# David-OConnor/molchanica

Hardware: AMD Instinct MI355X
Metric: MD atom-updates/sec (and steps/sec), 1M-atom solvated box (higher is better)
Workload: dtype f32

## Files before the change

### molchanica_amd/csrc/mdx_api.hip

```cpp
#include "mdx_comm.h"
#include <algorithm>
#include <atomic>
#include <chrono>
#include <cfloat>
#include <cmath>
#include <cstring>
#include <dlfcn.h>
#include <mutex>
#include <unordered_map>

static thread_local std::string g_last_error;
void mdx_set_error(const std::string& s) { g_last_error = s; }

static inline unsigned div_up(unsigned a, unsigned b) { return (a + b - 1) / b; }
static bool cut_on(float rc) { return rc > 0.f && std::isfinite(rc); }
static uint32_t f2u(float f) { uint32_t u; std::memcpy(&u, &f, 4); return u; }
static float u2f(uint32_t u) { float f; std::memcpy(&f, &u, 4); return f; }

#define FAIL(code, msg) do { mdx_set_error(msg); return (code); } while (0)

template <typename T>
static int upload_vec(T** dptr, const std::vector<T>& v, hipStream_t st) {
    if (*dptr) { (void)hipFree(*dptr); *dptr = nullptr; }
    HIP_TRY(hipMalloc((void**)dptr, std::max<size_t>(sizeof(T) * v.size(), 16)));
// ... 1277 lines not shown
    HIP_TRY(hipStreamSynchronize(h->stream));
    mdx_prof_collect(h);
    h->profile = enable != 0; h->profile_level = enable;
    if (enable) {
        h->stats.nb_ms_sum = h->stats.bonded_ms_sum = h->stats.integ_ms_sum = 0.0;
        h->stats.rebuild_ms_sum = h->stats.wall_ms_sum = 0.0;
        h->stats.nb_launches = h->stats.bonded_launches = h->stats.integ_launches = 0;
        if (h->dd) for (int k = 0; k < MDX_DIAG_PHASES; ++k) { h->dd->phase_ms[k] = 0.0; h->dd->phase_n[k] = 0; }
    }
    return MDX_OK;
}

extern "C" int mdx_get_skin(const mdx_handle* h, float* skin, int* tuning) {
    if (!h) FAIL(MDX_EPARAM, "null handle");
    if (skin) *skin = h->cfg.skin;
    if (tuning) *tuning = (h->skin_tune.on && h->skin_tune.phase < 4) ? 1 : 0;
    return MDX_OK;
}

extern "C" int mdx_pair_launch_info(const mdx_handle* h, uint32_t out[24]) {
    if (!h || !out) FAIL(MDX_EPARAM, "null argument");
    for (int k = 0; k < 8; ++k) { out[k] = h->pair_info_step[k]; out[8 + k] = h->pair_info_any[k]; }
    out[16] = h->inner_rebuilds; out[17] = h->inner_from_rebuild ? 1u : 0u; out[18] = h->water_step_launches; out[19] = h->water_step_mixed_launches;
    out[20] = (uint32_t)h->onepass_launches; out[21] = (uint32_t)h->onepass_violations; out[22] = 0u; out[23] = 0u;
    return MDX_OK;
}

extern "C" int mdx_get_stats(mdx_handle* h, mdx_stats* out) {
    if (!h || !out) FAIL(MDX_EPARAM, "null argument");
    HIP_TRY(hipSetDevice(h->device));
    HIP_TRY(hipStreamSynchronize(h->stream));
    mdx_prof_collect(h);
    h->stats.step_count = h->step_count; h->stats.rebuild_count = h->rebuild_count;
    h->stats.n_inner_cluster_pairs = 0; h->stats.prune_passes = 0;
    if (h->d.inner_count) {
        unsigned long long c[MDX_EPART + 1];
        HIP_TRY(hipSetDevice(h->device));
        HIP_TRY(hipMemcpyAsync(c, h->d.inner_count, sizeof(c), hipMemcpyDeviceToHost, h->stream));
        HIP_TRY(hipStreamSynchronize(h->stream));
        unsigned long long tot = 0;
        for (int k = 0; k < MDX_EPART; ++k) tot += c[k];
        h->stats.prune_passes = c[MDX_EPART];
        h->stats.n_inner_cluster_pairs = c[MDX_EPART] ? tot / c[MDX_EPART] : 0;
    }
    h->stats.n_owned = h->dd ? h->dd->n_owned : h->n_local;
    h->stats.n_ghost = h->dd ? h->dd->n_local - h->dd->n_owned : 0;
    h->stats.repartitions = h->dd ? h->dd->repartitions : 0;
// ... 300 lines not shown
```

### molchanica_amd/csrc/mdx_grid.hip

```cpp
#include "mdx_internal.h"
#include <atomic>
#include <chrono>
#include <algorithm>
#include <cfloat>
#include <cmath>

#define WAVE_LDS_SYNC()                                      \
    do {                                                     \
        __builtin_amdgcn_fence(__ATOMIC_SEQ_CST, "workgroup"); \
        __builtin_amdgcn_wave_barrier();                     \
    } while (0)

static inline unsigned div_up(unsigned a, unsigned b) { return (a + b - 1) / b; }

constexpr int SCAN_THREADS = 256;
constexpr int SCAN_ITEMS = 8;
constexpr int SCAN_TILE = SCAN_THREADS * SCAN_ITEMS;

__device__ __forceinline__ uint32_t block_exclusive_scan_256(uint32_t v, uint32_t* s_wave, uint32_t* total) {
    const int lane = threadIdx.x & 63, wave = threadIdx.x >> 6;
    uint32_t inc = v;
#pragma unroll
    for (int d = 1; d < 64; d <<= 1) {
        uint32_t t = __shfl_up(inc, d);
// ... 985 lines not shown
            if ((lane & 7) == 0 && newy != ent.y) entries[e0 + c * 8 + (lane >> 3)].y = newy;
            if (inner_on && (lane & 7) == 0) pin.entries_in[e0 + c * 8 + (lane >> 3)] = make_uint2(ent.x, newy_in);
        } else {
            const bool alive = (lane & 7) == 0 && ((newy >> 8) & 0xFFu) != 0u;
            const unsigned long long bal = __ballot(alive);
            if (alive) {
                const uint32_t rank = __popcll(bal & ((1ull << lane) - 1ull));
                entries[e0 + cnt.n_masked + wcur + rank] = make_uint2(ent.x, newy);
            }
            wcur += __popcll(bal);
            if (inner_on) {
                const bool alive_in = (lane & 7) == 0 && ((newy_in >> 8) & 0xFFu) != 0u;
                const unsigned long long bin = __ballot(alive_in);
                if (alive_in) pin.entries_in[e0 + cnt.n_masked + wcur_in + __popcll(bin & ((1ull << lane) - 1ull))] = make_uint2(ent.x, newy_in);
                wcur_in += __popcll(bin);
            }
        }
    }
    const uint32_t np_pad = (wcur + 7u) & ~7u;
    if (lane < (int)(np_pad - wcur)) entries[e0 + cnt.n_masked + wcur + lane] = make_uint2(null_cluster, 13u);
    if (inner_on) {
        const uint32_t nin_pad = (wcur_in + 7u) & ~7u;
        if (lane < (int)(nin_pad - wcur_in)) pin.entries_in[e0 + cnt.n_masked + wcur_in + lane] = make_uint2(null_cluster, 13u);
        if (lane == 0) pin.inner_nch[(size_t)t * 8] = nmc + (nin_pad >> 3);
    }
    const bool any_ghost = __any(ghost_hit);
    if (lane == 0) {
        counts[t].n_plain = np_pad;
        if (kept) atomicAdd(pc_slot(pair_count, t, 1), (unsigned long long)kept);
        if (tile_int) tile_int[t] = (!any_ghost && t * MDX_CL_PER_TILE < first_ghost_cluster) ? 1u : 0u;
    }
}

template <int W>
__global__ __launch_bounds__(W * 64) void prune_list_mw_kernel(uint32_t T, float r2, float shx, float shy, float shz,
                                                               const float4* __restrict__ posq, ListCounts* __restrict__ counts,
                                                               const uint32_t* __restrict__ entry_off, uint2* __restrict__ entries,
                                                               uint32_t null_cluster, unsigned long long* __restrict__ pair_count,
                                                               const uint32_t* __restrict__ rb_ctl, uint32_t* __restrict__ tile_int,
                                                               const uint8_t* __restrict__ cl_kind) {
    __shared__ float4 s_j[W][64];
    __shared__ uint32_t s_ghost;
    const int lane = threadIdx.x & 63, wave = __builtin_amdgcn_readfirstlane(threadIdx.x >> 6);
    uint32_t first_ghost_cluster = 0xFFFFFFFFu;
    if (rb_ctl) {
        T = __builtin_amdgcn_readfirstlane(rb_ctl[0]); null_cluster = T * MDX_CL_PER_TILE;
        first_ghost_cluster = __builtin_amdgcn_readfirstlane(rb_ctl[1]) * MDX_CL_PER_TILE;
// ... 953 lines not shown
    }
    const uint32_t T = h->T, S = h->S, NC = (T + 1) * MDX_CL_PER_TILE;
    {
        const TileOrderPlan plan = tile_order_plan(h, T);
        if (!res.classified) {
            h->tile_split = false; h->n_interior = 0;
            if (plan.split) MDX_TRY(mdx_classify_tiles(h, plan.lpt));
        }
        if (!res.ordered) {
            h->tile_lpt_on = false;
            if (plan.lpt) MDX_TRY(mdx_order_tiles_by_length(h, plan.grouped));
        }
    }
    h->list_valid = true;
    h->forces_valid = false;
    h->rebuild_count++; h->steps_since_rebuild = 0;
    mdx_dd_note_rebuild(h);
    h->inner_skin = h->inner_skin_auto > 0.f ? h->inner_skin_auto : c_inner_skin(h->cfg);
    h->dual_on = !h->dual_auto_off && mdx_nb_half(h) && prune && h->inner_skin > 0.f && h->inner_skin < h->cfg.skin &&
                 (h->n_vsites == 0 || h->vsites_convex);
    h->prune_pending = !(res.inner_built && h->dual_on);
    h->inner_from_rebuild = !h->prune_pending;
    if (h->inner_from_rebuild) ++h->inner_rebuilds;
    if (!d.inner_count) { ALLOC(d.inner_count, MDX_EPART + 8); HIP_TRY(hipMemsetAsync(d.inner_count, 0, sizeof(unsigned long long) * (MDX_EPART + 8), st)); }
    uint64_t nmask = (uint64_t)MC * 8;
    h->stats.n_atoms = N; h->stats.n_slots = S; h->stats.n_tiles = T; h->stats.n_clusters = NC;
    h->stats.n_list_entries = E; h->stats.n_masked_entries = nmask;
    h->stats.n_cluster_pairs = (mdx_nb_variant(h) >= 2) ? npairs : (uint64_t)E * 8;
    if (h->profile) {
        float ms = 0.f;
        HIP_TRY(hipEventRecord(e1, st)); HIP_TRY(hipEventSynchronize(e1));
        HIP_TRY(hipEventElapsedTime(&ms, e0, e1));
        h->stats.rebuild_ms_sum += ms;
        h->ev_pool.push_back(e0); h->ev_pool.push_back(e1);
    }
    return MDX_OK;
}

__global__ __launch_bounds__(1024) void lpt_order_kernel(uint32_t T, const ListCounts* __restrict__ counts, const uint32_t* __restrict__ is_int,
                                                         uint32_t* __restrict__ order, uint32_t group_tiles) {
    constexpr uint32_t NB = 8 * LPT_BUCKETS;
    __shared__ uint32_t s_hist[NB], s_cur[NB];
    for (uint32_t b = threadIdx.x; b < NB; b += blockDim.x) s_hist[b] = 0;
    __syncthreads();
    auto bucket = [&](uint32_t t) {
        const uint32_t nch = (counts[t].n_masked + counts[t].n_plain) >> 3;
// ... 143 lines not shown
```

### molchanica_amd/csrc/mdx_internal.h

```cpp
#pragma once
#include <hip/hip_runtime.h>
#include <stdint.h>
#include <chrono>
#include <string>
#include <vector>
#include "../../include/mdx.h"

#define MDX_TILE 64
#define MDX_CLUSTER 8
#define MDX_CL_PER_TILE 8
#define MDX_ACC_CONV 418.4f
#define MDX_KB 0.0019872041
#define MDX_INVALID 0xFFFFFFFFu
#define MDX_DUMMY_BASE 1.0e6f
#define MDX_DUMMY_STEP 64.0f
#define MDX_MAX_CHUNK 64
#define MDX_MAX_GROUPS 255

#define MDX_ESTRIDE 5
#define MDX_EPART 256
enum { EN_BOND = 0, EN_ANGLE, EN_DIHEDRAL, EN_LJ, EN_COUL, EN_LJ14, EN_COUL14, EN_KIN, EN_RECIP, EN_VIRIAL, EN_POSRE, EN_POSRE_VIR, EN_COUNT };

struct GridParams {
    float lo[3];
    float len[3];
    float inv_col[2];
// ... 270 lines not shown
        float dt_tuned = 0.f;
        std::chrono::steady_clock::time_point t0;
    } skin_tune;
    int chunk_s = -1;
    bool list_valid = false;
    bool forces_valid = false;
    bool in_slot_space = false;
    bool have_ext = false;
    uint64_t step_count = 0, rebuild_count = 0;
    bool profile = false; int profile_level = 0; bool prof_open = false;
    struct EvPair { hipEvent_t a, b; int kind; int tag; hipStream_t st; };
    int prof_tag = -1;
    uint32_t prof_seq = 0; bool prof_sampled = false;
    std::vector<EvPair> ev_pending;
    std::vector<hipEvent_t> ev_pool;
    mdx_stats stats{};
    int tstat_kind = 0; float tstat_temp = 300.f, tstat_tau = 1.f; uint32_t tstat_every = 10;
    int integrator = 0; float lang_gamma = 1.f, lang_temp = 300.f; uint64_t lang_seed = 0, lang_step = 0;
    int baro_kind = 0; float baro_p0 = 1.f, baro_tau = 5.f, baro_beta = 4.5e-5f; uint32_t baro_every = 25;
    double last_pressure = 0.0, last_mu = 1.0;
    bool force_zeroed = false;
    bool cons_full_kick = false;
    bool bonded_fused = false;
    uint32_t pair_info_step[8] = {}, pair_info_any[8] = {};
    bool bonded_deferred = false;
    uint64_t rng_state = 0;
    bool zero_com = false;
    uint32_t snap_every = 0; bool snap_vel = false;
    uint32_t snap_handlers[MDX_SNAP_HANDLERS] = {};
    double time_ps = 0.0;
    struct Snapshot { double time; uint64_t step; mdx_energies e; std::vector<float> pos, vel, frc; std::vector<mdx_hbond> hbonds; std::vector<float> between; uint32_t handler_mask = 0;
                      std::vector<double> foreign; };
    uint32_t water_first = 0, n_waters = 0, water_sites = 0;
    std::vector<uint8_t> hb_heavy; float hb_dmax = 2.5f, hb_angle_min = 120.f;
    std::vector<uint32_t> hb_donor_of;
    std::vector<uint32_t> h_bond_pairs;
    std::vector<Snapshot> snapshots;
    DeviceState d;
    StepCtl* h_ctl = nullptr;
    uint32_t ctl_seq = 0;
    uint32_t* h_rb = nullptr;
    uint32_t rb_seq = 0;
    uint32_t scan_gen = 0;
    bool cell_count_clean = false;
    bool slot_of_clean = false;
};
// ... 60 lines not shown
static inline bool mdx_nb_half(const mdx_handle* h) { return mdx_nb_variant(h) == 5; }
static inline uint32_t mdx_wpt8_below(const mdx_handle* h) {
    static const int env = [] { const char* e = std::getenv("MDX_WPT8_BELOW"); return e ? std::atoi(e) : -1; }();
    (void)h;
    return env >= 0 ? (uint32_t)env : 2048u;
}

#ifndef MDX_NB_WAVES
#define MDX_NB_WAVES 1
#endif
struct WptRule { int env; uint32_t wpt8_below; int decomposed; };
__host__ __device__ static inline int mdx_wpt_rule(const WptRule& r, uint32_t T) {
    if (r.env) return r.env;
    if (T >= 12000u) return r.decomposed ? 2 : 1;
    if (T >= (r.decomposed ? 8000u : 3000u)) return 2;
    return T < r.wpt8_below ? 8 : 4;
}
static inline WptRule mdx_wpt_rule_of(const mdx_handle* h) {
    static const int env = [] { const char* e = std::getenv("MDX_WPT"); return (e && (e[0] == '1' || e[0] == '2' || e[0] == '4' || e[0] == '8')) ? e[0] - '0' : 0; }();
    WptRule r; r.env = env; r.wpt8_below = mdx_wpt8_below(h); r.decomposed = (h->dd || h->n_local != h->N) ? 1 : 0;
    return r;
}
static inline int mdx_nb_wpt_half(const mdx_handle* h, uint32_t T) { return mdx_wpt_rule(mdx_wpt_rule_of(h), T); }

int mdx_build_constraints(mdx_handle* h, const mdx_system* s);
int mdx_remap_constraints(mdx_handle* h);
int mdx_launch_constrain_positions(mdx_handle* h, float dt, const uint32_t* d_gate, uint32_t* d_disp_out, uint32_t thr,
                                   uint32_t* d_prune_out = nullptr, bool skip_wstep = false);
int mdx_launch_constrain_velocities(mdx_handle* h, const uint32_t* d_gate, uint32_t thr);
bool mdx_water_step_ok(const mdx_handle* h);
bool mdx_water_step_mixed(const mdx_handle* h);
int mdx_launch_water_step(mdx_handle* h, int mode, float dt, const uint32_t* d_gate, uint32_t* d_disp_out, uint32_t thr, uint32_t* d_prune_out);
int mdx_launch_vsite_construct(mdx_handle* h, const uint32_t* d_gate, uint32_t thr);
int mdx_launch_constraint_virial(mdx_handle* h);
int mdx_check_box(const mdx_handle* h, const float* lo, const float* hi);
int mdx_launch_vsite_spread(mdx_handle* h, const uint32_t* d_gate, uint32_t thr);

int mdx_pme_setup(mdx_handle* h);
int mdx_pme_cu_split(const mdx_handle* h, const mdx_config* c);
int mdx_stream_create_masked(hipStream_t* s, int cus_per_xcd, bool complement);
int mdx_stream_unmask(mdx_handle* h);
void mdx_pme_destroy(mdx_handle* h);
int mdx_launch_pme(mdx_handle* h, bool energy, const uint32_t* d_gate, uint32_t thr);
int mdx_pme_fork(mdx_handle* h);
int mdx_pme_join(mdx_handle* h, const uint32_t* d_gate, uint32_t thr);

// ... 37 lines not shown
```

### molchanica_amd/csrc/mdx_nonbonded.hip

```cpp
#include "mdx_internal.h"
#include "mdx_bonded_dev.h"
#include "mdx_pair_dev.h"
#include <algorithm>
#include <cfloat>
#include <cstdlib>
#include <cstring>
#include <vector>

template <bool ENERGY, int COUL>
void launch_variant(mdx_handle* h, const NbArgs& a, bool geom, bool samecut);
#define NB_EXTERN(E, C) extern template void launch_variant<E, C>(mdx_handle*, const NbArgs&, bool, bool);
NB_EXTERN(false, CM_SHIFTED) NB_EXTERN(false, CM_RF) NB_EXTERN(false, CM_EWALD) NB_EXTERN(false, CM_SOFT)
NB_EXTERN(false, CM_EWALD_TAB)
NB_EXTERN(true, CM_SHIFTED) NB_EXTERN(true, CM_RF) NB_EXTERN(true, CM_EWALD) NB_EXTERN(true, CM_SOFT)
#undef NB_EXTERN

static bool cut_on(float rc) { return rc > 0.f && std::isfinite(rc); }
#define FAIL_NB(msg) do { mdx_set_error(msg); return MDX_EDEVICE; } while (0)

void mdx_fill_nb_params(const mdx_handle* h, NbParams& p, int* mode_out, bool* geom_out, bool* samecut_out) {
    const mdx_config& c = h->cfg;
    p.rc2_lj = cut_on(c.lj_cutoff) ? c.lj_cutoff * c.lj_cutoff : FLT_MAX;
    p.rc2_coul = cut_on(c.coulomb_cutoff) ? c.coulomb_cutoff * c.coulomb_cutoff : FLT_MAX;
    for (int d = 0; d < 3; ++d) p.shift[d] = h->per[d] ? (h->box_hi[d] - h->box_lo[d]) : 0.f;
    const bool ccut = cut_on(c.coulomb_cutoff);
    const float rc = c.coulomb_cutoff;
    p.alpha = c.ewald_alpha; p.soft2 = c.softening_sq;
    p.k_rf = 0.f; p.k_rf2 = 0.f; p.coul_shift = 0.f;
    p.alch_scale = h->alch_on ? (float)(1.0 - h->alch_lambda) : 1.0f;
    p.sc_alpha = h->alch_on ? h->sc_alpha : 0.f; p.sc_al = h->alch_on ? (float)(h->sc_alpha * h->alch_lambda) : 0.f;
    p.sc_sigmin = h->sc_sigma_min;
    int mode = CM_SHIFTED;
    switch (c.coulomb_mode) {
    case MDX_COULOMB_REACTION:
        mode = CM_RF;
        if (ccut) { p.k_rf = 1.0f / (2.0f * rc * rc * rc); p.k_rf2 = 2.0f * p.k_rf; p.coul_shift = 1.5f / rc; }
        break;
    case MDX_COULOMB_EWALD: mode = CM_EWALD; break;
// ... 140 lines not shown
```

### molchanica_amd/csrc/mdx_nonbonded_impl.h

```cpp
#pragma once
#include "mdx_internal.h"
#include "mdx_bonded_dev.h"
#include "mdx_pair_dev.h"
#include <algorithm>
#include <cfloat>
#include <cstdlib>
#include <type_traits>

constexpr int NB_WAVES = MDX_NB_WAVES;
#ifndef NB_ASM_PAIR
#define NB_ASM_PAIR 0
#endif
#ifndef NB_HALF_FLUSH
#define NB_HALF_FLUSH 0
#endif

template <bool BIAS, bool R2OUT>
__device__ __forceinline__ void pair_eval_asm(float xi, float yi, float zi, float qi, float sgi, float epi, const float4 pj,
                                              const float2 lj, float rc2, float bias, float& fx, float& fy, float& fz,
                                              float& g0, float& g1, float& g2, float& r2_out) {
    float dx, dy, dz, r2, t1, t2, t3, t4;
    if (BIAS) {
        asm volatile(
            "v_sub_f32 %[dy], %[yi], %[yj]\n\t"
            "v_sub_f32 %[dx], %[xi], %[xj]\n\t"
            "v_fma_f32 %[r2], %[dy], %[dy], %[bias]\n\t"
            "v_sub_f32 %[dz], %[zi], %[zj]\n\t"
            "v_fmac_f32 %[r2], %[dx], %[dx]\n\t"
            "v_fmac_f32 %[r2], %[dz], %[dz]\n\t"
            : [dx] "=&v"(dx), [dy] "=&v"(dy), [dz] "=&v"(dz), [r2] "=&v"(r2)
            : [xi] "v"(xi), [yi] "v"(yi), [zi] "v"(zi), [xj] "v"(pj.x), [yj] "v"(pj.y), [zj] "v"(pj.z), [bias] "v"(bias));
    } else {
// ... 124 lines not shown
        if (lane == 0) {
            double* q = a.energy + EN_COUNT + 8 + MDX_ESTRIDE * (blk & (MDX_EPART - 1));
            atomicAdd(q, 0.5 * elj); atomicAdd(q + 1, 0.5 * ecoul); atomicAdd(q + 2, 0.5 * evir);
        }
    }
}

template <int CTRL>
__device__ __forceinline__ float dpp_xadd(float v) {
    return v + __int_as_float(__builtin_amdgcn_update_dpp(0, __float_as_int(v), CTRL, 0xF, 0xF, true));
}

template <bool ENERGY, int COUL, bool GEOM, bool SAMECUT, int WPT, bool HALF, bool ALCH, int DUAL, int BW, bool STEP = false>
__device__ __forceinline__ void nb_cluster_body(const NbArgs& a, const bool owned_prune, float4 (*s_xyzq)[64], float2 (*s_lj)[64],
                                                float (*s_red)[3][64], float (*s_ownj)[64], float4 (*s_g)[64],
                                                unsigned long long (*s_mask)[64], const float4* __restrict__ etab = nullptr) {
    const int lane = threadIdx.x & 63, wave = __builtin_amdgcn_readfirstlane(threadIdx.x >> 6);
    constexpr int SPLIT = BW < WPT ? WPT / BW : 1;
    static_assert(SPLIT == 1 || HALF, "a tile split over workgroups returns its i-forces through atomics");
    constexpr int TPB = SPLIT > 1 ? 1 : BW / WPT;
    const uint32_t ntiles = a.tile_order ? a.t_count : a.T;
    const uint32_t nblocks = SPLIT > 1 ? ntiles * SPLIT : (ntiles + TPB - 1) / TPB;
    const uint32_t per_xcd = (nblocks + 7) >> 3;
    const uint32_t blk = a.xcd_interleave ? blockIdx.x : (blockIdx.x & 7u) * per_xcd + (blockIdx.x >> 3);
    if (blk >= nblocks) return;
    const int tib = SPLIT > 1 ? 0 : wave / WPT;
    const int part = SPLIT > 1 ? (int)(blk % SPLIT) * BW + wave : wave % WPT;
    const uint32_t tidx = SPLIT > 1 ? blk / SPLIT : blk * TPB + tib;
    const bool t_ok = tidx < ntiles;
    if (WPT == 1 && !t_ok) return;
    const uint32_t t = t_ok ? (a.tile_order ? __builtin_amdgcn_readfirstlane(a.tile_order[a.t_first + tidx]) : tidx) : a.T;
    const int ii = lane & 7, jj = lane >> 3;

    float xi[8], yi[8], zi[8], qi[8], sgi[8], epi[8], fx[8], fy[8], fz[8];
    if constexpr (STEP) {
        static_assert(HALF && !ENERGY && !ALCH && DUAL != 0, "one launch per step: half list, dual list");
        const uint32_t s = t * MDX_TILE + lane;
        const float4 Y = a.posq[s], Fp = a.st_fprev[s];
        const float4 x = step_pos(Y, Fp);
        if (part == 0 && t_ok) {
            float4 v = a.st_vel[s];
            float d2w = 0.f, pw = 0.f;
            bool viol = false;
            if (v.w != 0.f) {
                const float w = Fp.w, kdt = a.st_kick * a.st_dt * v.w;
                const float4 Fm = a.st_fnext[s];
                const float kx = w * Fp.x, ky = w * Fp.y, kz = w * Fp.z;
                const float sx_ = fmaf(a.st_dt, v.x, kx), sy_ = fmaf(a.st_dt, v.y, ky), sz_ = fmaf(a.st_dt, v.z, kz);
                v.x = fmaf(kdt, Fp.x, v.x); v.y = fmaf(kdt, Fp.y, v.y); v.z = fmaf(kdt, Fp.z, v.z);
                float path;
                const float4 r = a.ref[s];
// ... 70 lines not shown
    const uint32_t nmc = cnt.n_masked >> 3;
    const uint32_t nchunks = DUAL == 1 ? (t_ok ? a.inner_nch[t * 8 + part] : 0u) : (cnt.n_masked + cnt.n_plain) >> 3;
    const uint32_t mbase = a.mchunk_off[t_ok ? t : 0];
    float4* sx = s_xyzq[wave];
    float2* sl = s_lj[wave];
    double elj = 0.0, ecoul = 0.0, evir = 0.0, ecross = 0.0, edudl = 0.0;
    uint32_t own_bits = 0xFFu;
    if (ENERGY && !a.energy_all) {
        own_bits = 0;
#pragma unroll
        for (int ci = 0; ci < 8; ++ci)
            own_bits |= ((a.slot_flags[t * MDX_TILE + ci * MDX_CLUSTER + ii] >> 1) & 1u) << ci;
    }

    float4 nj = make_float4(0.f, 0.f, 0.f, 0.f), nf = nj;
    float2 nl = make_float2(0.f, 0.f);
    uint32_t ny = 13, njc = 0;
    float nown = 0.f;
    unsigned long long nmq = ~0ull;
    uint2 ent_n = make_uint2(0u, 13u);
    if ((uint32_t)part < nchunks) {
        const uint2 ent = entries[e0 + part * 8 + (lane >> 3)];
        if ((uint32_t)part < nmc) nmq = a.masks[(size_t)(mbase + part) * 64 + lane];
        if ((uint32_t)part + WPT < nchunks) ent_n = entries[e0 + (part + WPT) * 8 + (lane >> 3)];
        const uint32_t js = ent.x * MDX_CLUSTER + (lane & 7);
        nj = a.posq[js]; nl = a.lj[js]; ny = ent.y; njc = ent.x;
        if (STEP) nf = a.st_fprev[js];
        if (ENERGY && HALF) nown = a.energy_all ? 1.0f : (float)((a.slot_flags[js] >> 1) & 1u);
    }
    float* const fbase = reinterpret_cast<float*>(a.force);
    float4* const sg = s_g[HALF ? wave : 0];
    constexpr bool prune = DUAL == 2;
    uint32_t kept = 0;
#ifdef NB_HALF_STATS
    uint32_t dbg_jh = 0, dbg_ih = 0, dbg_q = 0, dbg_pairs = 0;
#endif
    const uint32_t c_first = nmc + ((uint32_t)part + WPT - nmc % WPT) % WPT;
    uint32_t wcur = 0;
    if (HALF && NB_HALF_FLUSH) __builtin_amdgcn_s_waitcnt(0x0F70);
    const float rc2_s = __builtin_bit_cast(float, __builtin_amdgcn_readfirstlane(__builtin_bit_cast(int, a.p.rc2_lj)));
    auto chunk_pass = [&](auto masked_tag, const uint32_t c_begin, const uint32_t c_end) __attribute__((always_inline)) {
    constexpr bool MASKED_CHUNK = decltype(masked_tag)::value;
    for (uint32_t c = c_begin; c < c_end; c += WPT) {
        const uint32_t cur_y = ny, cur_jc = njc;
        constexpr bool masked = MASKED_CHUNK;
        if (masked) s_mask[wave][lane] = nmq;
        if (ENERGY && HALF) s_ownj[wave][lane] = nown;
        if (HALF && NB_HALF_FLUSH) {
            const bool live = ((ny >> 8) & 0xFFu) != 0u;
            sg[lane] = make_float4(0.f, 0.f, 0.f, __uint_as_float(live ? njc * MDX_CLUSTER + (uint32_t)ii : t * MDX_TILE + lane));
        }
        {
            const uint32_t code = ny & 31u;
            const int kx = (int)(code % 3u) - 1, ky = (int)((code / 3u) % 3u) - 1, kz = (int)(code / 9u) - 1;
            if (STEP) nj = step_pos(nj, nf);
            nj.x += (float)kx * a.p.shift[0];
            nj.y += (float)ky * a.p.shift[1];
            nj.z += (float)kz * a.p.shift[2];
            sx[lane] = nj;
            sl[lane] = nl;
        }
        WAVE_LDS_SYNC();
        if (c + WPT < nmc) nmq = a.masks[(size_t)(mbase + c + WPT) * 64 + lane];
        if (c + WPT < nchunks) {
            const uint32_t js = ent_n.x * MDX_CLUSTER + (lane & 7);
            nj = a.posq[js]; nl = a.lj[js]; ny = ent_n.y; njc = ent_n.x;
            if (STEP) nf = a.st_fprev[js];
            if (ENERGY && HALF) nown = a.energy_all ? 1.0f : (float)((a.slot_flags[js] >> 1) & 1u);
            if (c + 2 * WPT < nchunks) ent_n = entries[e0 + (c + 2 * WPT) * 8 + (lane >> 3)];
        }
        float celj = 0.f, cecoul = 0.f, cevir = 0.f, cecross = 0.f, cedudl = 0.f;
        uint32_t newy = cur_y & 0xFFu;
#pragma unroll 1
        for (int e = 0; e < 8; ++e) {
            const float4 pj = sx[e * 8 + jj];
            const float2 lj = sl[e * 8 + jj];
            const uint32_t im = (__builtin_amdgcn_readlane(cur_y, e * 8) >> 8) & 0xFFu;
            if (im == 0) continue;
            uint32_t newm = 0;
            const int x8 = MASKED_CHUNK ? (int)(~(uint32_t)reinterpret_cast<const uint8_t*>(&s_mask[wave][lane])[e]) : 0;
            float g[3] = {0.f, 0.f, 0.f};
            float wj = 0.f;
            if (ENERGY && HALF) wj = 0.5f * s_ownj[wave][e * 8 + jj];
#pragma unroll
            for (int ci = 0; ci < 8; ++ci) {
                if (im & (1u << ci)) {
                    float e1 = 0.f, e2 = 0.f, e3 = 0.f, e4 = 0.f, e5 = 0.f;
                    const float bias = MASKED_CHUNK ? __int_as_float((x8 << (31 - ci)) >> 31) : 0.f;
                    float r2v = 0.f;
                    constexpr bool ASM_PAIR = NB_ASM_PAIR && !ENERGY && COUL == CM_SHIFTED && !GEOM && SAMECUT && HALF && !ALCH;
                    if constexpr (ASM_PAIR)
                        pair_eval_asm<MASKED_CHUNK, prune>(xi[ci], yi[ci], zi[ci], qi[ci], sgi[ci], epi[ci], pj, lj, rc2_s, bias, fx[ci], fy[ci], fz[ci],
// ... 35 lines not shown
                    g[d] = dpp_xadd<0x4E>(g[d]);
                    g[d] = dpp_xadd<0x141>(g[d]);
                }
                if (ii < 3) {
                    const float v = ii == 0 ? g[0] : (ii == 1 ? g[1] : g[2]);
                    if (NB_HALF_FLUSH) reinterpret_cast<float*>(sg)[(e * 8 + jj) * 4 + ii] = -v;
#ifdef NB_EXP_NOATOMIC
                    else if (v == 1.2345e30f) unsafeAtomicAdd(fbase + (size_t)__builtin_amdgcn_readlane(cur_jc, e * 8) * (MDX_CLUSTER * 4) + jj * 4 + ii, -v);
#else
                    else unsafeAtomicAdd(fbase + (size_t)__builtin_amdgcn_readlane(cur_jc, e * 8) * (MDX_CLUSTER * 4) + jj * 4 + ii, -v);
#endif
                }
            }
        }
        if (ENERGY) { elj += (double)celj; ecoul += (double)cecoul; evir += (double)cevir; ecross += (double)cecross; edudl += (double)cedudl; }
        if (prune) {
            if (masked) {
                if (ii == 0) a.entries_in[e0 + c * 8 + jj] = make_uint2(cur_jc, newy);
            } else {
                const bool alive = ii == 0 && (newy >> 8) != 0u;
                const unsigned long long bal = __ballot(alive);
                if (alive) {
                    const uint32_t k = wcur + (uint32_t)__popcll(bal & ((1ull << lane) - 1ull));
                    a.entries_in[e0 + (c_first + (k >> 3) * WPT) * 8 + (k & 7u)] = make_uint2(cur_jc, newy);
                }
                wcur += (uint32_t)__popcll(bal);
            }
        }
        WAVE_LDS_SYNC();
        if (HALF && NB_HALF_FLUSH) {
            __builtin_amdgcn_s_waitcnt(0x0F70);
            const float* const sgf = reinterpret_cast<const float*>(sg);
#pragma unroll
            for (int k = 0; k < 3; ++k) {
                const uint32_t fidx = (uint32_t)(k * 64 + lane), atom = (fidx * 171u) >> 9, comp = fidx - 3u * atom;
                const uint32_t slot = __float_as_uint(sgf[atom * 4 + 3]);
                unsafeAtomicAdd(fbase + (size_t)slot * 4 + comp, sgf[atom * 4 + comp]);
            }
        }
    }
    };
#ifndef NB_SPLIT_MASKED
#define NB_SPLIT_MASKED 1
#endif
    if (NB_SPLIT_MASKED) {
        const uint32_t c_mid = c_first < nchunks ? c_first : nchunks;
        chunk_pass(std::true_type{}, (uint32_t)part, c_mid);
        chunk_pass(std::false_type{}, c_mid, nchunks);
    } else chunk_pass(std::true_type{}, (uint32_t)part, nchunks);
    float ox = 0.f, oy = 0.f, oz = 0.f;
#pragma unroll
    for (int ci = 0; ci < 8; ++ci) {
        float x = fx[ci], y = fy[ci], z = fz[ci];
#pragma unroll
        for (int m = 8; m < 64; m <<= 1) {
            x += __shfl_xor(x, m); y += __shfl_xor(y, m); z += __shfl_xor(z, m);
        }
        if (jj == ci) { ox = x; oy = y; oz = z; }
    }
    float* const fi = fbase + (size_t)(t * MDX_TILE + lane) * 4;
    if (prune && t_ok) {
        const uint32_t nfull = (wcur + 7u) >> 3;
        if ((uint32_t)lane < nfull * 8u - wcur) {
            const uint32_t k = wcur + (uint32_t)lane;
            a.entries_in[e0 + (c_first + (k >> 3) * WPT) * 8 + (k & 7u)] = make_uint2(a.T * MDX_CL_PER_TILE, 13u);
        }
        if (lane == 0) a.inner_nch[t * 8 + part] = nfull ? c_first + (nfull - 1u) * WPT + 1u : nmc;
    }
    if (prune) {
        if (!STEP && part == 0 && t_ok && (owned_prune || !(a.slot_flags[t * MDX_TILE + lane] & 2u))) {
            const uint32_t s = t * MDX_TILE + lane;
            if (a.path) {
                const float4 x = a.posq[s], r = a.ref[s];
                const float dx = x.x - r.x, dy = x.y - r.y, dz = x.z - r.z;
                a.path[s] = 0.f; a.dprune[s] = __builtin_sqrtf(dx * dx + dy * dy + dz * dz);
            } else a.ref[s].w = 0.f;
        }
        if (lane == 0 && kept) atomicAdd(a.inner_count + ((blk * BW + wave) & (MDX_EPART - 1)), (unsigned long long)kept);
        if (lane == 0 && blk == 0 && wave == 0) atomicAdd(a.inner_count + MDX_EPART, 1ull);
#ifdef NB_HALF_STATS
        if (lane == 0) {
            atomicAdd(a.inner_count + MDX_EPART + 1, (unsigned long long)dbg_jh); atomicAdd(a.inner_count + MDX_EPART + 2, (unsigned long long)dbg_ih);
            atomicAdd(a.inner_count + MDX_EPART + 3, (unsigned long long)dbg_q); atomicAdd(a.inner_count + MDX_EPART + 4, (unsigned long long)kept);
            atomicAdd(a.inner_count + MDX_EPART + 5, (unsigned long long)dbg_pairs);
        }
#endif
    }
    if (WPT > 1) {
        s_red[wave][0][lane] = ox; s_red[wave][1][lane] = oy; s_red[wave][2][lane] = oz;
        __syncthreads();
// ... 76 lines not shown
    static_assert(!FB || DUAL != 0, "the bonded workgroups ride with the dual-list launches");
    constexpr int BW = SPLIT > 1 ? WPT / SPLIT : (WPT > NB_WAVES ? WPT : NB_WAVES);
    if ((DUAL == 4 || DUAL == 6 || FB) && blockIdx.x >= a.pair_grid) {
        if (DUAL == 1 || DUAL == 2) {
            const bool want_prune = (a.force_prune | *a.prune_flag) != 0u || (a.prune_flag2 && *a.prune_flag2 != 0u);
            if (want_prune != (DUAL == 2)) return;
        }
        bonded_workgroup<STEP>(a, blockIdx.x - a.pair_grid, BW * 64);
        return;
    }
    __shared__ float4 s_xyzq[BW][64];
    __shared__ float2 s_lj[BW][64];
    __shared__ float s_red[WPT > 1 ? BW : 1][3][64];
    __shared__ float s_ownj[(ENERGY && HALF) ? BW : 1][64];
    __shared__ float4 s_g[HALF ? BW : 1][64];
    __shared__ unsigned long long s_mask[BW][64];
    extern __shared__ float4 s_dyn_etab[];
    const float4* etab = nullptr;
    if (COUL == CM_EWALD_TAB && !ENERGY && !ALCH) {
        for (uint32_t k = threadIdx.x; k < a.p.etab_n; k += BW * 64) s_dyn_etab[k] = a.p.etab[k];
        __syncthreads();
        etab = reinterpret_cast<const float4*>(reinterpret_cast<const char*>(s_dyn_etab) - ((EWALD_TAB_CBITS >> a.p.etab_shift) << 4));
    }
    if (DUAL == 0) {
        nb_cluster_body<ENERGY, COUL, GEOM, SAMECUT, WPT, HALF, ALCH, 0, BW>(a, true, s_xyzq, s_lj, s_red, s_ownj, s_g, s_mask, etab);
    } else {
        const bool owned_prune = (a.force_prune | *a.prune_flag) != 0u;
        const bool want_prune = owned_prune || (a.prune_flag2 && *a.prune_flag2 != 0u);
        if (DUAL >= 3) {
#if NB_MERGED_NOINLINE
            if (want_prune) nb_cluster_body_call<ENERGY, COUL, GEOM, SAMECUT, WPT, HALF, ALCH, 2, BW>(a, owned_prune, s_xyzq, s_lj, s_red, s_ownj, s_g, s_mask, etab);
            else nb_cluster_body_call<ENERGY, COUL, GEOM, SAMECUT, WPT, HALF, ALCH, 1, BW>(a, owned_prune, s_xyzq, s_lj, s_red, s_ownj, s_g, s_mask, etab);
#else
            if (want_prune) nb_cluster_body<ENERGY, COUL, GEOM, SAMECUT, WPT, HALF, ALCH, 2, BW, STEP>(a, owned_prune, s_xyzq, s_lj, s_red, s_ownj, s_g, s_mask, etab);
            else nb_cluster_body<ENERGY, COUL, GEOM, SAMECUT, WPT, HALF, ALCH, 1, BW, STEP>(a, owned_prune, s_xyzq, s_lj, s_red, s_ownj, s_g, s_mask, etab);
#endif
        } else {
            if (want_prune != (DUAL == 2)) return;
            nb_cluster_body<ENERGY, COUL, GEOM, SAMECUT, WPT, HALF, ALCH, DUAL == 2 ? 2 : 1, BW>(a, owned_prune, s_xyzq, s_lj, s_red, s_ownj, s_g, s_mask, etab);
        }
    }
}

template <bool ENERGY, int COUL>
void launch_variant(mdx_handle* h, const NbArgs& a, bool geom, bool samecut) {
    const int var = mdx_nb_variant(h);
    int wpt = 1;
    const bool half = var == 5;
    if (var == 2) wpt = (a.T < mdx_wpt8_below(h)) ? 8 : 4;
    if (half) wpt = mdx_nb_wpt_half(h, a.T);
    if (var == 4) wpt = 4;
    const uint32_t bw = std::max(wpt, NB_WAVES);
    const uint32_t tpb = (var == 1) ? NB_WAVES : bw / wpt;
    const uint32_t nblocks = ((a.tile_order ? a.t_count : a.T) + tpb - 1) / tpb;
    const uint32_t grid = ((nblocks + 7) / 8) * 8;
    if (nblocks == 0) return;
    dim3 g(grid), b(bw * 64);
    static const uint32_t lds_pad_env = [] { const char* e = std::getenv("MDX_NB_LDS_PAD"); return e ? (uint32_t)std::atoi(e) : 0u; }();
    const uint32_t lds_pad = ((h->pme_on && h->pme_overlap && !ENERGY) ? lds_pad_env : 0u) +
                             ((COUL == CM_EWALD_TAB && !ENERGY) ? a.p.etab_n * (uint32_t)sizeof(float4) : 0u);
    static const bool dual_merged = [] { const char* e = std::getenv("MDX_DUAL_MERGED"); return !(e && e[0] == '0'); }();
    static const bool merge_all = [] { const char* e = std::getenv("MDX_DUAL_MERGED"); return !(e && (e[0] == '0' || e[0] == '1')); }();
    static const int split_env = [] { const char* e = std::getenv("MDX_TILE_SPLIT"); return e ? (e[0] == '0' ? 0 : 1) : -1; }();
    const bool split2 = split_env >= 0 ? split_env == 1 : (a.tile_order ? a.t_count : a.T) < 1024u;
    static const bool fb_all = [] { const char* e = std::getenv("MDX_FUSE_BONDED"); return e && e[0] == '2'; }();
    auto note = [&](int dual, int w, int split, int fb) {
        uint32_t* const o = a.inner ? h->pair_info_step : h->pair_info_any;
        o[0] = (uint32_t)w; o[1] = (uint32_t)dual; o[2] = half ? 1u : 0u; o[3] = (uint32_t)COUL; o[4] = ENERGY ? 1u : 0u;
        o[5] = (uint32_t)split; o[6] = (uint32_t)fb; o[7] = a.tile_order ? a.t_count : a.T;
    };
#define NB_STEP(G, S)                                                                                                 \
    do {                                                                                                               \
        if constexpr (!ENERGY && !G && COUL != CM_SOFT) {                                                              \
            if (wpt == 1 && half && a.inner) {                                                                         \
                hipLaunchKernelGGL((nb_cluster_kernel<false, COUL, false, S, 1, true, false, 5>), g, b, lds_pad, h->stream, a); \
                note(5, 1, 1, 0);                                                                                      \
            } else if (wpt == 8 && half && a.inner && split2) {             \
                NbArgs af = a;                                                                                         \
                const uint32_t nb2 = (a.tile_order ? a.t_count : a.T) * 2u;                                            \
                af.pair_grid = ((nb2 + 7) / 8) * 8;                                                                    \
// ... 67 lines not shown
```

### molchanica_amd/csrc/mdx_pair_dev.h

```cpp
#pragma once
#include "mdx_internal.h"

struct NbParams;
void mdx_fill_nb_params(const mdx_handle* h, NbParams& p, int* mode_out, bool* geom_out, bool* samecut_out);

#define WAVE_LDS_SYNC()                                        \
    do {                                                       \
        __builtin_amdgcn_fence(__ATOMIC_SEQ_CST, "workgroup"); \
        __builtin_amdgcn_wave_barrier();                       \
    } while (0)

struct NbArgs {
    uint32_t T;
    const float4* posq; const float2* lj;
    const ListCounts* counts; const uint32_t* entry_off; const uint32_t* mchunk_off;
    const uint2* entries; const unsigned long long* masks;
    float4* force; double* energy;
    const uint8_t* slot_flags;
    NbParams p;
    const uint32_t* gate; uint32_t thr_bits;
    uint32_t inner;
    uint32_t force_prune;
    const uint32_t* prune_flag;
    float rin2;
    uint2* entries_in;
    uint32_t* inner_nch;
    float4* ref; unsigned long long* inner_count;
    float* path; float* dprune;
    uint32_t xcd_interleave;
    const uint32_t* tile_order; uint32_t t_first, t_count;
    const uint32_t* prune_flag2;
    uint32_t energy_all;
    uint32_t pair_grid, b_S;
    const uint32_t* b_role_off; const RoleRec* b_roles; const float4* b_prm;
    BondedParams b_p;
    const float4* st_fprev; float4* st_yout; float4* st_fnext; float4* st_vel;
    float st_dt, st_path_thr;
    uint32_t st_last;
    float st_grant;
    float st_kick;
    uint32_t* st_disp_out;
    uint32_t* st_prune_out;
    uint32_t* st_viol;
};

enum { CM_SHIFTED = 0, CM_RF = 1, CM_EWALD = 2, CM_SOFT = 3,
       CM_EWALD_TAB = 4 };

#define EWALD_TAB_C 4.0f
#define EWALD_TAB_CBITS 0x40800000u
#define EWALD_TAB_MAX 1024u

template <bool ENERGY, int COUL, bool GEOM, bool SAMECUT, bool BRANCHY, bool HALF = false, bool ALCH = false, bool NANMASK = false>
__device__ __forceinline__ void pair_eval(float xi, float yi, float zi, float qi, float sgi, float epi,
                                          const float4 pj, const float2 lj, bool allowed, const NbParams& p,
                                          float& fx, float& fy, float& fz, float& elj, float& ecoul,
                                          float* g = nullptr, float* evir = nullptr, float* ecross = nullptr,
                                          float r2bias = 0.f, float* r2_out = nullptr, float* edudl = nullptr,
                                          const float4* __restrict__ etab = nullptr) {
    static_assert(!NANMASK || BRANCHY, "the NaN-coded exclusion needs the early-out");
    const float dx = xi - pj.x, dy = yi - pj.y, dz = zi - pj.z;
    const float r2 = NANMASK ? __builtin_fmaf(dz, dz, __builtin_fmaf(dx, dx, __builtin_fmaf(dy, dy, r2bias)))
                             : dx * dx + dy * dy + dz * dz;
    if (NANMASK) allowed = true;
    if (r2_out) *r2_out = r2;
    const bool in_lj = (r2 < p.rc2_lj) && allowed;
// ... 76 lines not shown
```

### molchanica_amd/md_state.py

```python
from __future__ import annotations

import ctypes as C
import os

import numpy as np

from ._abi import (CCommDiag, CHBond, CConfig, CEnergies, CStats, CSystem, FORCE, MDX_EDEVICE, MDX_ENAN, MDX_EOOM,
                   MDX_EPARAM, MDX_OK, POS, VEL, MdConfig, MdSystem)

_HERE = os.path.dirname(os.path.abspath(__file__))
LIB_PATH = os.environ.get("MDX_LIB") or os.path.join(_HERE, "libmdx.so")


class ParamError(ValueError):
    """The reference's `ParamError { descrip }` (src/md/mod.rs:967)."""


class DeviceError(RuntimeError):
    """HIP/device failure (MDX_EDEVICE / MDX_EOOM); the reference degrades to its CPU path here
    (src/util.rs:1072-1119) — this library has none and says so loudly."""


class BlowUpError(FloatingPointError):
    """Non-finite state (MDX_ENAN); cf. the stop criteria at sol_shrinking_box.rs:776-789."""
# ... 425 lines not shown

    def flush_snapshot_queues(self):
        _check(load_library().mdx_flush_snapshot_queues(self._h))

    @property
    def time_ps(self) -> float:
        return float(load_library().mdx_time_ps(self._h))

    def profile(self, enable=True):
        _check(load_library().mdx_profile(self._h, int(enable)))

    def stats(self) -> dict:
        s = CStats()
        _check(load_library().mdx_get_stats(self._h, C.byref(s)))
        return s.as_dict()

    def pair_launch_info(self) -> dict:
        out = (C.c_uint32 * 24)()
        _check(load_library().mdx_pair_launch_info(self._h, out))
        keys = ("waves_per_tile", "dual", "half", "coulomb", "energy", "workgroups_per_tile", "bonded_workgroups", "tiles")
        return {"step": dict(zip(keys, (int(v) for v in out[0:8]))), "any": dict(zip(keys, (int(v) for v in out[8:16]))),
                "inner_lists_from_rebuilds": int(out[16]), "last_rebuild_wrote_the_inner_list": bool(out[17]),
                "water_step_launches": int(out[18]), "water_step_mixed_launches": int(out[19]),
                "one_launch_steps": int(out[20]), "kicks_beyond_grant": int(out[21])}

    def skin(self):
        v, t = C.c_float(), C.c_int()
        _check(load_library().mdx_get_skin(self._h, C.byref(v), C.byref(t)))
        return float(v.value), bool(t.value)

    def computation_time(self) -> float:
        return float(self.stats()["wall_ms_sum"])

    def comm_init(self, unique_id: bytes, rank: int, world: int):
        assert len(unique_id) == 128
        _check(load_library().mdx_comm_init(self._h, bytes(unique_id), int(rank), int(world)))

    def comm_init_fabric(self, fabric: "Fabric", rank: int):
        self._fabric = fabric
        _check(load_library().mdx_comm_init_fabric(self._h, fabric.ptr, int(rank)))

    def comm_init_shm(self, name: str, rank: int, world: int):
        _check(load_library().mdx_comm_init_shm(self._h, name.encode(), int(rank), int(world)))

    def comm_init_null(self, rank: int, world: int):
        _check(load_library().mdx_comm_init_null(self._h, int(rank), int(world)))

# ... 147 lines not shown
```

Measured before the change: 2.022 billion.

## Split tail tiles of LPT-ordered nonbonded list across multiple waves

```diff
diff --git a/molchanica_amd/csrc/mdx_api.hip b/molchanica_amd/csrc/mdx_api.hip
--- a/molchanica_amd/csrc/mdx_api.hip
+++ b/molchanica_amd/csrc/mdx_api.hip
@@ -1323,7 +1323,7 @@
     if (!h || !out) FAIL(MDX_EPARAM, "null argument");
     for (int k = 0; k < 8; ++k) { out[k] = h->pair_info_step[k]; out[8 + k] = h->pair_info_any[k]; }
     out[16] = h->inner_rebuilds; out[17] = h->inner_from_rebuild ? 1u : 0u; out[18] = h->water_step_launches; out[19] = h->water_step_mixed_launches;
-    out[20] = (uint32_t)h->onepass_launches; out[21] = (uint32_t)h->onepass_violations; out[22] = 0u; out[23] = 0u;
+    out[20] = (uint32_t)h->onepass_launches; out[21] = (uint32_t)h->onepass_violations; out[22] = h->pair_info_tail[0]; out[23] = h->pair_info_tail[1];
     return MDX_OK;
 }
 
diff --git a/molchanica_amd/csrc/mdx_grid.hip b/molchanica_amd/csrc/mdx_grid.hip
--- a/molchanica_amd/csrc/mdx_grid.hip
+++ b/molchanica_amd/csrc/mdx_grid.hip
@@ -1031,7 +1031,7 @@
     if (inner_on) {
         const uint32_t nin_pad = (wcur_in + 7u) & ~7u;
         if (lane < (int)(nin_pad - wcur_in)) pin.entries_in[e0 + cnt.n_masked + wcur_in + lane] = make_uint2(null_cluster, 13u);
-        if (lane == 0) pin.inner_nch[(size_t)t * 8] = nmc + (nin_pad >> 3);
+        if (lane < 8) pin.inner_nch[(size_t)t * 8 + lane] = nmc + (nin_pad >> 3);
     }
     const bool any_ghost = __any(ghost_hit);
     if (lane == 0) {
@@ -2031,6 +2031,8 @@
     h->prune_pending = !(res.inner_built && h->dual_on);
     h->inner_from_rebuild = !h->prune_pending;
     if (h->inner_from_rebuild) ++h->inner_rebuilds;
+    h->tail_w = 0; h->tail_tiles = 0;
+    if (h->dual_on && h->tile_lpt_on && h->tile_lpt_grouped && !h->alch_on) mdx_tail_plan(h, T, &h->tail_w, &h->tail_tiles);
     if (!d.inner_count) { ALLOC(d.inner_count, MDX_EPART + 8); HIP_TRY(hipMemsetAsync(d.inner_count, 0, sizeof(unsigned long long) * (MDX_EPART + 8), st)); }
     uint64_t nmask = (uint64_t)MC * 8;
     h->stats.n_atoms = N; h->stats.n_slots = S; h->stats.n_tiles = T; h->stats.n_clusters = NC;
diff --git a/molchanica_amd/csrc/mdx_internal.h b/molchanica_amd/csrc/mdx_internal.h
--- a/molchanica_amd/csrc/mdx_internal.h
+++ b/molchanica_amd/csrc/mdx_internal.h
@@ -2,6 +2,8 @@
 #include <hip/hip_runtime.h>
 #include <stdint.h>
 #include <chrono>
+#include <cstdlib>
+#include <cstring>
 #include <string>
 #include <vector>
 #include "../../include/mdx.h"
@@ -318,6 +320,8 @@
     bool force_zeroed = false;
     bool cons_full_kick = false;
     bool bonded_fused = false;
+    uint32_t tail_w = 0, tail_tiles = 0;
+    uint32_t pair_info_tail[2] = {};
     uint32_t pair_info_step[8] = {}, pair_info_any[8] = {};
     bool bonded_deferred = false;
     uint64_t rng_state = 0;
@@ -424,6 +428,33 @@
     return r;
 }
 static inline int mdx_nb_wpt_half(const mdx_handle* h, uint32_t T) { return mdx_wpt_rule(mdx_wpt_rule_of(h), T); }
+#define MDX_WPT_TAIL_DEFAULT_W 4u
+#define MDX_WPT_TAIL_DEFAULT_DEN 8u
+static inline void mdx_tail_plan(const mdx_handle* h, uint32_t T, uint32_t* w_out, uint32_t* tiles_out) {
+    struct TailEnv { int set; uint32_t w, den; };
+    static const TailEnv env = [] {
+        TailEnv r{0, 0u, 0u};
+        const char* e = std::getenv("MDX_WPT_TAIL");
+        if (!e || !e[0]) return r;
+        r.set = 1;
+        const uint32_t w = (uint32_t)std::atoi(e);
+        const char* s = std::strchr(e, '/');
+        const uint32_t den = s ? (uint32_t)std::atoi(s + 1) : 8u;
+        if ((w == 2u || w == 4u) && den >= 1u) { r.w = w; r.den = den; }
+        return r;
+    }();
+    *w_out = 0; *tiles_out = 0;
+    if (h->dd || h->n_local != h->N || mdx_nb_wpt_half(h, T) != 1) return;
+    if (const char* e = std::getenv("MDX_ONEPASS")) { if (e[0] == '2') return; }
+    uint32_t w = 0, den = 0;
+    if (env.set) { w = env.w; den = env.den; }
+    else if (T >= 12000u && !h->pme_on) { w = MDX_WPT_TAIL_DEFAULT_W; den = MDX_WPT_TAIL_DEFAULT_DEN; }
+    if (w < 2u) return;
+    const uint32_t group = (T + 7u) >> 3;
+    const uint32_t tiles = den == 1u ? group : group / den;
+    if (!tiles) return;
+    *w_out = w; *tiles_out = tiles;
+}
 
 int mdx_build_constraints(mdx_handle* h, const mdx_system* s);
 int mdx_remap_constraints(mdx_handle* h);
diff --git a/molchanica_amd/csrc/mdx_nonbonded.hip b/molchanica_amd/csrc/mdx_nonbonded.hip
--- a/molchanica_amd/csrc/mdx_nonbonded.hip
+++ b/molchanica_amd/csrc/mdx_nonbonded.hip
@@ -14,6 +14,18 @@
 NB_EXTERN(false, CM_EWALD_TAB)
 NB_EXTERN(true, CM_SHIFTED) NB_EXTERN(true, CM_RF) NB_EXTERN(true, CM_EWALD) NB_EXTERN(true, CM_SOFT)
 #undef NB_EXTERN
+
+#ifdef NB_DRAIN_TRACE
+uint4* g_mdx_drain = nullptr; size_t g_mdx_drain_cap = 0; uint32_t g_mdx_drain_n = 0; int g_mdx_drain_on = 0;
+extern "C" int mdx_debug_drain_trace(mdx_handle* h, int on, uint32_t* out, uint32_t cap_waves) {
+    HIP_TRY(hipStreamSynchronize(h->stream));
+    g_mdx_drain_on = on;
+    if (!out || !g_mdx_drain) return 0;
+    const uint32_t n = std::min(g_mdx_drain_n, cap_waves);
+    HIP_TRY(hipMemcpy(out, g_mdx_drain, sizeof(uint4) * 2 * (size_t)n, hipMemcpyDeviceToHost));
+    return (int)n;
+}
+#endif
 
 static bool cut_on(float rc) { return rc > 0.f && std::isfinite(rc); }
 #define FAIL_NB(msg) do { mdx_set_error(msg); return MDX_EDEVICE; } while (0)
diff --git a/molchanica_amd/csrc/mdx_nonbonded_impl.h b/molchanica_amd/csrc/mdx_nonbonded_impl.h
--- a/molchanica_amd/csrc/mdx_nonbonded_impl.h
+++ b/molchanica_amd/csrc/mdx_nonbonded_impl.h
@@ -8,6 +8,9 @@
 #include <type_traits>
 
 constexpr int NB_WAVES = MDX_NB_WAVES;
+#ifdef NB_DRAIN_TRACE
+extern uint4* g_mdx_drain; extern size_t g_mdx_drain_cap; extern uint32_t g_mdx_drain_n; extern int g_mdx_drain_on;
+#endif
 #ifndef NB_ASM_PAIR
 #define NB_ASM_PAIR 0
 #endif
@@ -178,11 +181,24 @@
     const uint32_t ntiles = a.tile_order ? a.t_count : a.T;
     const uint32_t nblocks = SPLIT > 1 ? ntiles * SPLIT : (ntiles + TPB - 1) / TPB;
     const uint32_t per_xcd = (nblocks + 7) >> 3;
-    const uint32_t blk = a.xcd_interleave ? blockIdx.x : (blockIdx.x & 7u) * per_xcd + (blockIdx.x >> 3);
-    if (blk >= nblocks) return;
+    constexpr bool TAIL = WPT == 1 && HALF && DUAL != 0 && !STEP && BW == 1;
+    const bool tail_on = TAIL && a.tail_w > 1u;
+    const uint32_t blk = (a.xcd_interleave || tail_on) ? blockIdx.x : (blockIdx.x & 7u) * per_xcd + (blockIdx.x >> 3);
+    if (!tail_on && blk >= nblocks) return;
     const int tib = SPLIT > 1 ? 0 : wave / WPT;
-    const int part = SPLIT > 1 ? (int)(blk % SPLIT) * BW + wave : wave % WPT;
-    const uint32_t tidx = SPLIT > 1 ? blk / SPLIT : blk * TPB + tib;
+    int part = SPLIT > 1 ? (int)(blk % SPLIT) * BW + wave : wave % WPT;
+    uint32_t tidx = SPLIT > 1 ? blk / SPLIT : blk * TPB + tib;
+    uint32_t wv = WPT;
+    if (tail_on) {
+        const uint32_t xcd = blockIdx.x & 7u, u = blockIdx.x >> 3;
+        tidx = xcd * a.tail_group + u;
+        if (u >= a.tail_head) {
+            const uint32_t v = u - a.tail_head;
+            wv = a.tail_w;
+            part = (int)(v & (wv - 1u));
+            tidx = xcd * a.tail_group + a.tail_head + (v >> (wv == 4u ? 2 : 1));
+        }
+    }
     const bool t_ok = tidx < ntiles;
     if (WPT == 1 && !t_ok) return;
     const uint32_t t = t_ok ? (a.tile_order ? __builtin_amdgcn_readfirstlane(a.tile_order[a.t_first + tidx]) : tidx) : a.T;
@@ -299,7 +315,7 @@
     if ((uint32_t)part < nchunks) {
         const uint2 ent = entries[e0 + part * 8 + (lane >> 3)];
         if ((uint32_t)part < nmc) nmq = a.masks[(size_t)(mbase + part) * 64 + lane];
-        if ((uint32_t)part + WPT < nchunks) ent_n = entries[e0 + (part + WPT) * 8 + (lane >> 3)];
+        if ((uint32_t)part + wv < nchunks) ent_n = entries[e0 + (part + wv) * 8 + (lane >> 3)];
         const uint32_t js = ent.x * MDX_CLUSTER + (lane & 7);
         nj = a.posq[js]; nl = a.lj[js]; ny = ent.y; njc = ent.x;
         if (STEP) nf = a.st_fprev[js];
@@ -312,13 +328,13 @@
 #ifdef NB_HALF_STATS
     uint32_t dbg_jh = 0, dbg_ih = 0, dbg_q = 0, dbg_pairs = 0;
 #endif
-    const uint32_t c_first = nmc + ((uint32_t)part + WPT - nmc % WPT) % WPT;
+    const uint32_t c_first = nmc + (TAIL ? (((uint32_t)part + wv - (nmc & (wv - 1u))) & (wv - 1u)) : ((uint32_t)part + WPT - nmc % WPT) % WPT);
     uint32_t wcur = 0;
     if (HALF && NB_HALF_FLUSH) __builtin_amdgcn_s_waitcnt(0x0F70);
     const float rc2_s = __builtin_bit_cast(float, __builtin_amdgcn_readfirstlane(__builtin_bit_cast(int, a.p.rc2_lj)));
     auto chunk_pass = [&](auto masked_tag, const uint32_t c_begin, const uint32_t c_end) __attribute__((always_inline)) {
     constexpr bool MASKED_CHUNK = decltype(masked_tag)::value;
-    for (uint32_t c = c_begin; c < c_end; c += WPT) {
+    for (uint32_t c = c_begin; c < c_end; c += wv) {
         const uint32_t cur_y = ny, cur_jc = njc;
         constexpr bool masked = MASKED_CHUNK;
         if (masked) s_mask[wave][lane] = nmq;
@@ -338,13 +354,13 @@
             sl[lane] = nl;
         }
         WAVE_LDS_SYNC();
-        if (c + WPT < nmc) nmq = a.masks[(size_t)(mbase + c + WPT) * 64 + lane];
-        if (c + WPT < nchunks) {
+        if (c + wv < nmc) nmq = a.masks[(size_t)(mbase + c + wv) * 64 + lane];
+        if (c + wv < nchunks) {
             const uint32_t js = ent_n.x * MDX_CLUSTER + (lane & 7);
             nj = a.posq[js]; nl = a.lj[js]; ny = ent_n.y; njc = ent_n.x;
             if (STEP) nf = a.st_fprev[js];
             if (ENERGY && HALF) nown = a.energy_all ? 1.0f : (float)((a.slot_flags[js] >> 1) & 1u);
-            if (c + 2 * WPT < nchunks) ent_n = entries[e0 + (c + 2 * WPT) * 8 + (lane >> 3)];
+            if (c + 2 * wv < nchunks) ent_n = entries[e0 + (c + 2 * wv) * 8 + (lane >> 3)];
         }
         float celj = 0.f, cecoul = 0.f, cevir = 0.f, cecross = 0.f, cedudl = 0.f;
         uint32_t newy = cur_y & 0xFFu;
@@ -426,7 +442,7 @@
                 const unsigned long long bal = __ballot(alive);
                 if (alive) {
                     const uint32_t k = wcur + (uint32_t)__popcll(bal & ((1ull << lane) - 1ull));
-                    a.entries_in[e0 + (c_first + (k >> 3) * WPT) * 8 + (k & 7u)] = make_uint2(cur_jc, newy);
+                    a.entries_in[e0 + (c_first + (k >> 3) * wv) * 8 + (k & 7u)] = make_uint2(cur_jc, newy);
                 }
                 wcur += (uint32_t)__popcll(bal);
             }
@@ -467,9 +483,9 @@
         const uint32_t nfull = (wcur + 7u) >> 3;
         if ((uint32_t)lane < nfull * 8u - wcur) {
             const uint32_t k = wcur + (uint32_t)lane;
-            a.entries_in[e0 + (c_first + (k >> 3) * WPT) * 8 + (k & 7u)] = make_uint2(a.T * MDX_CL_PER_TILE, 13u);
-        }
-        if (lane == 0) a.inner_nch[t * 8 + part] = nfull ? c_first + (nfull - 1u) * WPT + 1u : nmc;
+            a.entries_in[e0 + (c_first + (k >> 3) * wv) * 8 + (k & 7u)] = make_uint2(a.T * MDX_CL_PER_TILE, 13u);
+        }
+        if (lane == 0) a.inner_nch[t * 8 + part] = nfull ? c_first + (nfull - 1u) * wv + 1u : nmc;
     }
     if (prune) {
         if (!STEP && part == 0 && t_ok && (owned_prune || !(a.slot_flags[t * MDX_TILE + lane] & 2u))) {
@@ -592,6 +608,9 @@
         __syncthreads();
         etab = reinterpret_cast<const float4*>(reinterpret_cast<const char*>(s_dyn_etab) - ((EWALD_TAB_CBITS >> a.p.etab_shift) << 4));
     }
+#ifdef NB_DRAIN_TRACE
+    const unsigned long long drain_t0 = wall_clock64();
+#endif
     if (DUAL == 0) {
         nb_cluster_body<ENERGY, COUL, GEOM, SAMECUT, WPT, HALF, ALCH, 0, BW>(a, true, s_xyzq, s_lj, s_red, s_ownj, s_g, s_mask, etab);
     } else {
@@ -609,11 +628,23 @@
             if (want_prune != (DUAL == 2)) return;
             nb_cluster_body<ENERGY, COUL, GEOM, SAMECUT, WPT, HALF, ALCH, DUAL == 2 ? 2 : 1, BW>(a, owned_prune, s_xyzq, s_lj, s_red, s_ownj, s_g, s_mask, etab);
         }
+#ifdef NB_DRAIN_TRACE
+        if (DUAL == 3 && a.drain) {
+            __builtin_amdgcn_s_waitcnt(0);
+            const unsigned long long t1 = wall_clock64();
+            if ((threadIdx.x & 63u) == 0u) {
+                uint4* const o = a.drain + 2 * ((size_t)blockIdx.x * BW + (threadIdx.x >> 6));
+                o[0] = make_uint4((uint32_t)drain_t0, (uint32_t)(drain_t0 >> 32), (uint32_t)t1, (uint32_t)(t1 >> 32));
+                o[1] = make_uint4(__builtin_amdgcn_s_getreg(4 | (31 << 11)), __builtin_amdgcn_s_getreg(20 | (31 << 11)), want_prune ? 1u : 0u, 1u);
+            }
+        }
+#endif
     }
 }
 
 template <bool ENERGY, int COUL>
-void launch_variant(mdx_handle* h, const NbArgs& a, bool geom, bool samecut) {
+void launch_variant(mdx_handle* h, const NbArgs& a_in, bool geom, bool samecut) {
+    NbArgs a = a_in;
     const int var = mdx_nb_variant(h);
     int wpt = 1;
     const bool half = var == 5;
@@ -626,6 +657,32 @@
     const uint32_t grid = ((nblocks + 7) / 8) * 8;
     if (nblocks == 0) return;
     dim3 g(grid), b(bw * 64);
+    if (half && wpt == 1 && a.inner && !ENERGY && !a.st_fprev && h->tail_w > 1u && h->tile_lpt_on && a.tile_order == h->d.tile_lpt && !a.xcd_interleave) {
+        a.tail_group = (a.T + 7u) >> 3;
+        const uint32_t tail = std::min(h->tail_tiles, a.tail_group);
+        a.tail_w = h->tail_w; a.tail_head = a.tail_group - tail;
+        g = dim3(8u * (a.tail_head + a.tail_w * tail));
+    }
+    if (a.inner) {
+        uint32_t n_tail = 0;
+        for (uint32_t x = 0; a.tail_w && x < 8u; ++x) {
+            const uint32_t in_range = a.T > x * a.tail_group ? std::min(a.T - x * a.tail_group, a.tail_group) : 0u;
+            n_tail += in_range > a.tail_head ? in_range - a.tail_head : 0u;
+        }
+        h->pair_info_tail[0] = a.tail_w; h->pair_info_tail[1] = n_tail;
+    }
+#ifdef NB_DRAIN_TRACE
+    if (a.inner && g_mdx_drain_on) {
+        const size_t want = (size_t)g.x * bw * 2;
+        if (want > g_mdx_drain_cap) {
+            if (g_mdx_drain) (void)hipFree(g_mdx_drain);
+            (void)hipMalloc((void**)&g_mdx_drain, sizeof(uint4) * want);
+            g_mdx_drain_cap = want;
+        }
+        (void)hipMemsetAsync(g_mdx_drain, 0, sizeof(uint4) * want, h->stream);
+        a.drain = g_mdx_drain; g_mdx_drain_n = (uint32_t)(g.x * bw);
+    }
+#endif
     static const uint32_t lds_pad_env = [] { const char* e = std::getenv("MDX_NB_LDS_PAD"); return e ? (uint32_t)std::atoi(e) : 0u; }();
     const uint32_t lds_pad = ((h->pme_on && h->pme_overlap && !ENERGY) ? lds_pad_env : 0u) +
                              ((COUL == CM_EWALD_TAB && !ENERGY) ? a.p.etab_n * (uint32_t)sizeof(float4) : 0u);
diff --git a/molchanica_amd/csrc/mdx_pair_dev.h b/molchanica_amd/csrc/mdx_pair_dev.h
--- a/molchanica_amd/csrc/mdx_pair_dev.h
+++ b/molchanica_amd/csrc/mdx_pair_dev.h
@@ -42,6 +42,10 @@
     uint32_t* st_disp_out;
     uint32_t* st_prune_out;
     uint32_t* st_viol;
+    uint32_t tail_w, tail_head, tail_group;
+#ifdef NB_DRAIN_TRACE
+    uint4* drain;
+#endif
 };
 
 enum { CM_SHIFTED = 0, CM_RF = 1, CM_EWALD = 2, CM_SOFT = 3,
diff --git a/molchanica_amd/md_state.py b/molchanica_amd/md_state.py
--- a/molchanica_amd/md_state.py
+++ b/molchanica_amd/md_state.py
@@ -471,7 +471,8 @@
         return {"step": dict(zip(keys, (int(v) for v in out[0:8]))), "any": dict(zip(keys, (int(v) for v in out[8:16]))),
                 "inner_lists_from_rebuilds": int(out[16]), "last_rebuild_wrote_the_inner_list": bool(out[17]),
                 "water_step_launches": int(out[18]), "water_step_mixed_launches": int(out[19]),
-                "one_launch_steps": int(out[20]), "kicks_beyond_grant": int(out[21])}
+                "one_launch_steps": int(out[20]), "kicks_beyond_grant": int(out[21]),
+                "tail": {"waves_per_tile": int(out[22]), "tiles": int(out[23])}}
 
     def skin(self):
         v, t = C.c_float(), C.c_int()
```

New measurement: 2.086 billion, median of 6. +3.2%, better.
